# BowieHsu/tensorflow_ocr

Measured on AMD Instinct MI355X. Metric: images/sec training, 512x512 ICDAR, VGG-16 EAST, batch 32, 1/2/4/8 GPU, higher is better.
Workload: dtype f16; 1 GPU; VGG-16 model_vgg + dice loss train step, 512x512, batch 32 per GPU, f16 storage / f32 accumulate, Adam+EMA; global_batch=32, parallelism=dp1

## Files before the change

### include/ocr_hip.h

```cpp
#ifndef OCR_HIP_H_
#define OCR_HIP_H_

#include <stddef.h>
#include <stdint.h>

#ifdef __cplusplus
extern "C" {
#endif

#define OCR_ABI_VERSION 7

enum {
  OCR_OK = 0,
  OCR_ERR_INVALID_ARG = -1,
  OCR_ERR_UNSUPPORTED = -2,
  OCR_ERR_HIP = -3,
  OCR_ERR_WORKSPACE = -4,
  OCR_ERR_RCCL = -5
};

int ocr_abi_version(void);
const char* ocr_status_string(int status);
const char* ocr_storage_dtype(void);
uint32_t ocr_crc32c(const void* data, size_t n, uint32_t seed);
// ... 43 lines not shown

int ocr_conv2d_bnred_tail_f16(const ocr_conv_desc* d, const void* x, const void* w_kc, void* y, void* partial,
                              const void* bn_y, const void* bn_mean, const void* bn_invstd,
                              const void* tail_out, const void* tail_mask_bits, const void* sub_grad, void* stream);

int ocr_conv2d_pw_bnaddrelu_f16(const ocr_conv_desc* d, const void* prev_y, const void* prev_scale,
                                const void* prev_shift, const void* shortcut, const void* sc_scale,
                                const void* sc_shift, void* x_out, void* mask_bits, const void* w_kc, void* y,
                                void* stats, void* stream);
int ocr_conv2d_pw_bnrelu_f16(const ocr_conv_desc* d, const void* prev_y, const void* prev_scale, const void* prev_shift,
                             void* x_out, const void* w_kc, void* y, void* stats, void* stream);
int ocr_conv2d_pw_bnbwd_bnred_f16(const ocr_conv_desc* d, const void* dz, const void* y_above, const void* coef_a,
                                  const void* coef_b, const void* coef_c, void* dy_out, const void* w_kc, void* dx,
                                  void* partial, const void* bn_y, const void* bn_scale, const void* bn_shift,
                                  const void* bn_mean, const void* bn_invstd, int bn_relu, void* stream);
int ocr_conv2d_pw_bnbwd_tail_f16(const ocr_conv_desc* d, const void* dz, const void* y_above, const void* coef_a,
                                 const void* coef_b, const void* coef_c, const void* relu_shift, void* dy_out,
                                 const void* w_kc, void* dx, void* partial, const void* bn_y, const void* bn_mean,
                                 const void* bn_invstd, const void* tail_out, const void* tail_mask_bits,
                                 const void* sub_grad, void* stream);

int ocr_conv2d_first_f16(int n, int h, int w, int cout, const void* x4,
                         const void* w_first, const void* bias, int flags,
                         void* y, void* stats, void* stream);
int ocr_conv2d_first_num_mtiles(int n, int h, int w);

int ocr_conv2d_wgrad_f16(const ocr_conv_desc* d, const void* x, const void* dy,
                         void* dw_hwio_f32, void* workspace, size_t ws_bytes,
                         void* stream);
size_t ocr_conv2d_wgrad_workspace(const ocr_conv_desc* d);
int ocr_conv2d_wgrad_slabs_f16(const ocr_conv_desc* d, const void* x, const void* dy, void* workspace, size_t ws_bytes,
                               void* stream);
int ocr_conv2d_wgrad_reduce_f32(const ocr_conv_desc* d, const void* workspace, void* dw_hwio_f32, void* stream);
int ocr_conv2d_wgrad_guest_room(const ocr_conv_desc* d);

int ocr_conv2d_first_wgrad_f16(int n, int h, int w, int cout, const void* x4,
                               const void* dy, void* dw_hwio_f32,
                               void* workspace, size_t ws_bytes, void* stream);
int ocr_conv2d_first_wgrad_bn_f16(int n, int h, int w, int cout, const void* x4, const void* da, const void* bn_y,
                                  const void* w_first, const void* bn_shift, const void* coef_a, const void* coef_b,
                                  const void* coef_c, int relu, void* dw, void* workspace, size_t ws_bytes,
                                  void* stream);
int ocr_conv2d_first_bn_relu_f16(int n, int h, int w, int cout, const void* x4, const void* w_first,
                                 const void* scale, const void* shift, int relu, void* a, void* stream);
size_t ocr_conv2d_first_wgrad_workspace(int n, int h, int w, int cout);

int ocr_conv2d_stem_num_mtiles(int n, int h, int w);
int ocr_pack_weights_stem_f16(const void* w_hwio_f32, int cout, void* w_stem, void* stream);
int ocr_conv2d_stem_f16(int n, int h, int w, int cout, const void* x4, const void* w_stem,
                        const void* bias, int flags, void* y, void* stats, void* stream);
size_t ocr_conv2d_stem_wgrad_workspace(int n, int h, int w, int cout);
int ocr_conv2d_stem_wgrad_f16(int n, int h, int w, int cout, const void* x4, const void* dy,
                              void* dw_hwio_f32, void* workspace, size_t ws_bytes, void* stream);
int ocr_conv2d_stem_wgrad_bn_f16(int n, int h, int w, int cout, const void* x4, const void* da, const void* bn_y,
                                 const void* bn_shift, const void* coef_a, const void* coef_b, const void* coef_c,
                                 int relu, void* dw, void* workspace, size_t ws_bytes, void* stream);
int ocr_pack_weights_f16(const void* w_hwio_f32, int taps, int cin, int cout, void* w_kc,
                         void* w_ck, void* stream);
int ocr_pack_weights_first_f16(const void* w_hwio_f32, int cout, void* w_first, void* stream);
size_t ocr_conv2d_first_moments_workspace(void);
int ocr_conv2d_first_moments_f16(int n, int h, int w, int cout, const void* x4, const void* w_first, void* stats_row,
                                 void* workspace, size_t ws_bytes, void* stream);
int ocr_conv2d_first_moments_keep_f16(int n, int h, int w, int cout, const void* x4, const void* w_first,
                                      void* stats_row, void* moments_f64, void* workspace, size_t ws_bytes, void* stream);
size_t ocr_pack_weights_batch_table_bytes(int n);
int ocr_pack_weights_batch_table(int n, const void* const* w_hwio_f32, const int* taps, const int* cin,
// ... 344 lines not shown
```

### tensorflow_ocr_amd/csrc/conv_first.hip

```cpp
#include "common.h"
#include "conv_epilogue.h"

namespace {

constexpr int HW = 36;

struct FirstP {
  int n, h, w, cout, tiles_x, tiles_y, m_tiles, flags;
};

__device__ __forceinline__ void load_halo4(const half_t* __restrict__ x4, char* halo, int img, int h,
                                           int w, int iy0, int ix0) {
  for (int i = threadIdx.x; i < 10 * HW; i += 256) {
    const int hy = i / HW, hx = i - hy * HW;
    const int iy = iy0 + hy, ix = ix0 + hx;
    u32x2 v = {0u, 0u};
    if (iy >= 0 && iy < h && ix >= 0 && ix < w)
      v = *reinterpret_cast<const u32x2*>(x4 + (((size_t)img * h + iy) * w + ix) * 4);
    *reinterpret_cast<u32x2*>(halo + i * 8) = v;
  }
}

__device__ __forceinline__ void first_weights(const half_t* __restrict__ wf, int cout, int co0, int lane,
                                              half8_t (&a)[3][2]) {
  const int r = lane & 31, hh = lane >> 5;
#pragma unroll
  for (int ky = 0; ky < 3; ++ky)
#pragma unroll
    for (int i = 0; i < 2; ++i)
      a[ky][i] = *reinterpret_cast<const half8_t*>(wf + ((size_t)(ky * cout + co0 + i * 32 + r)) * 16 + 8 * hh);
}

__device__ __forceinline__ void first_mfma(const char* halo, const half8_t (&a)[3][2], int wave, int lane,
                                           f32x16 (&acc)[2][2]) {
  const int r = lane & 31, hh = lane >> 5;
#pragma unroll
  for (int i = 0; i < 2; ++i)
#pragma unroll
    for (int t = 0; t < 2; ++t)
#pragma unroll
      for (int e = 0; e < 16; ++e) acc[i][t][e] = 0.f;
#pragma unroll
  for (int ky = 0; ky < 3; ++ky) {
#pragma unroll
    for (int t = 0; t < 2; ++t) {
      const int ty = wave * 2 + t;
      const char* src = halo + ((ty + ky) * HW + r + 2 * hh) * 8;
      half4_t lo = *reinterpret_cast<const half4_t*>(src);
      half4_t hi = *reinterpret_cast<const half4_t*>(src + 8);
      half8_t b = {lo[0], lo[1], lo[2], lo[3], hi[0], hi[1], hi[2], hi[3]};
#pragma unroll
      for (int i = 0; i < 2; ++i)
        acc[i][t] = OCR_MFMA_32x32x16(a[ky][i], b, acc[i][t], 0, 0, 0);
    }
  }
}

struct FirstAct {
  const float *scale, *shift;
  int relu;
};

template <bool BNAPPLY>
// ... 556 lines not shown
```

### tensorflow_ocr_amd/csrc/conv_wgrad.hip

```cpp
#include "common.h"
#include <stdlib.h>

namespace ocr_detail {
int wgrad_pw_splits(const ocr_conv_desc* d);
int wgrad_pw_launch(const ocr_conv_desc* d, const void* x, const void* dy, void* slab, hipStream_t st);
bool wgrad_pw_is_256x256(const ocr_conv_desc* d);
}

namespace {

typedef short short4v __attribute__((__vector_size__(4 * sizeof(short))));
typedef __attribute__((address_space(3))) short4v* lds_s4_ptr;

struct WgP {
  int n, h, w, cin, oh, ow, cout, kh, kw, stride, dil, pt, pl;
  int tiles_x, tiles_y, m_tiles, HT, WT, splits, tiles_per_split, nci, nco;
};

OCR_DIAG_DECLARE(ocr_diag_wgrad)

constexpr int TILE_H = 8;
constexpr int TILE_W = 32;
constexpr int CIB = 64;
constexpr int COB = 64;
constexpr int XSTR = CIB * 2 + 16;
constexpr int DSTR = COB * 2 + 16;

__device__ __forceinline__ half8_t tr_pair(const char* base, int second_off) {
  short4v lo = __builtin_amdgcn_ds_read_tr16_b64_v4i16((lds_s4_ptr)(base));
  short4v hi = __builtin_amdgcn_ds_read_tr16_b64_v4i16((lds_s4_ptr)(base + second_off));
  typedef short short8v __attribute__((ext_vector_type(8)));
  short8v v = {lo[0], lo[1], lo[2], lo[3], hi[0], hi[1], hi[2], hi[3]};
  return __builtin_bit_cast(half8_t, v);
// ... 317 lines not shown
    }
    if (more) store_tile(buf ^ 1);
    __syncthreads();
  }

  OCR_DIAG_END(ocr_diag_wgrad)
#pragma unroll
  for (int t = 0; t < MAXTAPS; ++t) {
    if (t < ntaps) {
      float* dst = slab + (((size_t)(split * KG + kgrp) * ntaps + t) * p.cin + ci0 + ciw * 32 + 4 * g) * p.cout +
                   co0 + cow * 32 + li;
      if (ci0 + ciw * 32 < p.cin && co0 + cow * 32 < p.cout) {
#pragma unroll
        for (int i = 0; i < 2; ++i)
#pragma unroll
          for (int j = 0; j < 2; ++j)
#pragma unroll
            for (int e = 0; e < 4; ++e) dst[(size_t)(i * 16 + e) * p.cout + j * 16] = acc[t][i][j][e];
      }
    }
  }
}


template <int N> struct WgIC { static constexpr int value = N; };
template <typename F>
__device__ __forceinline__ void static_for4(F&& f) {
  f(WgIC<0>{});
  f(WgIC<1>{});
  f(WgIC<2>{});
  f(WgIC<3>{});
}

template <int MAXTAPS, int COB2>
__global__ __launch_bounds__(256) void wgrad3_kernel(Wg2P p, const half_t* __restrict__ x,
                                                      const half_t* __restrict__ dy,
                                                      float* __restrict__ slab) {
  constexpr int NT = 256;
  static_assert(COB2 == 128 || COB2 == 64, "cout block");
  constexpr int NJ = COB2 / 32;
  constexpr int DSTR2 = COB2 * 2 + 32;
  constexpr int DCH = COB2 / 8;
  constexpr int NDY = 128 * DCH / NT;
  constexpr int PPP = NT / DCH;
  constexpr int XPP = NT / 8;
  constexpr int NXMAX = (224 + XPP - 1) / XPP;
  extern __shared__ __attribute__((aligned(16))) char smem[];
  const int halo_px = p.HT * p.WT;
  const int halo_bytes = halo_px * X2STR;
  const int stage_bytes = halo_bytes + 128 * DSTR2;

  const int tid = threadIdx.x;
  const int lane = tid & 63, wave = tid >> 6;
  const int ciw = wave >> 1, cow = wave & 1;
  const int li = lane & 15, g = lane >> 4;
  const int q = li >> 2, pp = li & 3;

  int bid = blockIdx.x;
  if (p.xcd_swizzle) bid = (bid & 7) * (int)(gridDim.x >> 3) + (bid >> 3);
  const int cob = bid % p.nco;
  bid /= p.nco;
  const int cib = bid % p.nci;
  const int split = bid / p.nci;
  const int ci0 = cib * CIB, co0 = cob * COB2;
  const int ntaps = p.kh * p.kw;

  f32x4 acc[MAXTAPS][2][NJ];
#pragma unroll
  for (int t = 0; t < MAXTAPS; ++t)
#pragma unroll
    for (int i = 0; i < 2; ++i)
#pragma unroll
      for (int j = 0; j < NJ; ++j) acc[t][i][j] = f32x4{0.f, 0.f, 0.f, 0.f};

  const int a_lane = ((4 * g + q) * p.stride) * X2STR + (ciw * 32 + 4 * pp) * 2;
  const int a_half = 16 * p.stride * X2STR;
  const int b_lane = (4 * g + q) * DSTR2 + (cow * (COB2 / 2) + 4 * pp) * 2;
  const int b_half = 16 * DSTR2;

  const int mt_begin = split * p.tiles_per_split;
  int mt_end = mt_begin + p.tiles_per_split;
  if (mt_end > p.m_tiles) mt_end = p.m_tiles;

  constexpr unsigned OOB = 0xfffffff0u;
  constexpr int WT_ = 34, HALO_PX = 6 * WT_;
  const int xc = tid & 7;
  int hxv[NXMAX];
  unsigned relx[NXMAX];
#pragma unroll
  for (int u = 0; u < NXMAX; ++u) {
    const int hp = u * XPP + (tid >> 3);
    const int hy = hp / WT_, hx = hp - hy * WT_;
    hxv[u] = (hp < HALO_PX && ci0 + xc * 8 < p.cin) ? hx : 0x40000000;
    relx[u] = (unsigned)(((hy * p.w + hx) * p.cin + ci0 + xc * 8) * 2);
  }
  const int dc = tid % DCH, dprow = tid / DCH;
  int colv[2];
#pragma unroll
  for (int h2 = 0; h2 < 2; ++h2) colv[h2] = (co0 + dc * 8 < p.cout) ? (h2 * 16) % 32 + dprow : 0x40000000;
  const unsigned reld = (unsigned)((dprow * p.cout + co0 + dc * 8) * 2);

  int l_mt = mt_begin;
  int l_txi = l_mt % p.tiles_x, l_tyi = (l_mt / p.tiles_x) % p.tiles_y, l_img = l_mt / (p.tiles_x * p.tiles_y);
  int s_ix0 = 0, s_orgx = 0, s_ox0 = 0, s_orgd = 0;
  __amdgpu_buffer_rsrc_t xrs, drs;
  auto load_setup = [&]() {
    s_ix0 = l_txi * TILE_W - p.pl;
    s_orgx = ((l_tyi * T2_H - p.pt) * p.w + s_ix0) * p.cin * 2;
    s_ox0 = l_txi * TILE_W;
    s_orgd = ((l_tyi * T2_H) * p.ow + s_ox0) * p.cout * 2;
    xrs = __builtin_amdgcn_make_buffer_rsrc(const_cast<half_t*>(x) + (size_t)l_img * p.h * p.w * p.cin, 0,
                                            p.h * p.w * p.cin * 2, 0x00020000);
    drs = __builtin_amdgcn_make_buffer_rsrc(const_cast<half_t*>(dy) + (size_t)l_img * p.oh * p.ow * p.cout, 0,
                                            p.oh * p.ow * p.cout * 2, 0x00020000);
  };
  auto load_advance = [&]() {
    if (l_mt + 1 < mt_end) {
      ++l_mt;
      if (++l_txi == p.tiles_x) {
        l_txi = 0;
        if (++l_tyi == p.tiles_y) {
          l_tyi = 0;
          ++l_img;
        }
      }
    }
    load_setup();
  };
  u32x4 xr[NXMAX], dr[NDY];
  unsigned offp = 0;
  auto load_half = [&](int hh) {
    const int k = hh >> 1;
    if (k >= NXMAX + NDY) return;
    if (k < NXMAX) {
      if (!(hh & 1)) {
        const int ix = hxv[k] + s_ix0;
        offp = (unsigned)ix < (unsigned)p.w ? relx[k] + (unsigned)s_orgx : OOB;
      } else {
        xr[k] = __builtin_bit_cast(u32x4, __builtin_amdgcn_raw_buffer_load_b128(xrs, offp, 0, 0));
      }
    } else {
      const int u = k - NXMAX;
      if (!(hh & 1)) {
        const int ox = colv[((u * PPP) >> 4) & 1] + s_ox0;
        offp = (unsigned)ox < (unsigned)p.ow ? reld + (unsigned)(s_orgd + (((u * PPP) >> 5) * p.ow + ((u * PPP) & 31)) * p.cout * 2) : OOB;
      } else {
        dr[u] = __builtin_bit_cast(u32x4, __builtin_amdgcn_raw_buffer_load_b128(drs, offp, 0, 0));
      }
    }
  };
  auto store_piece = [&](int buf, int k) {
    char* xh = smem + buf * stage_bytes;
    if (k < NXMAX) {
      if (k * XPP + XPP <= HALO_PX || k * XPP + (tid >> 3) < HALO_PX)
        *reinterpret_cast<u32x4*>(xh + (k * XPP + (tid >> 3)) * X2STR + xc * 16) = xr[k];
    } else if (k < NXMAX + NDY) {
      const int u = k - NXMAX;
      *reinterpret_cast<u32x4*>(xh + halo_bytes + (u * PPP + dprow) * DSTR2 + dc * 16) = dr[u];
    }
  };
  auto load_tile = [&]() {
#pragma unroll
    for (int hh = 0; hh < 2 * (NXMAX + NDY); ++hh) load_half(hh);
  };
  auto store_tile = [&](int buf) {
#pragma unroll
    for (int k = 0; k < NXMAX + NDY; ++k) store_piece(buf, k);
  };

  OCR_DIAG_BEGIN()
  if (mt_begin < mt_end) {
    load_setup();
    load_tile();
    store_tile(0);
    load_advance();
    load_tile();
  }
  __syncthreads();
#ifndef WG3_ABL
#define WG3_ABL 0
#endif
  typedef short short8v __attribute__((ext_vector_type(8)));
  short4v al[4][2], ah[4][2], bl[2][NJ], bh[2][NJ];
  auto rd = [&](const char* a) { return __builtin_amdgcn_ds_read_tr16_b64_v4i16((lds_s4_ptr)(a)); };
  auto frag = [&](const short4v& lo, const short4v& hi) {
    short8v v = __builtin_shufflevector(lo, hi, 0, 1, 2, 3, 4, 5, 6, 7);
    return __builtin_bit_cast(half8_t, v);
  };
  auto read_b1 = [&](int set, const char* dyt, int ty, int k) {
    if constexpr ((WG3_ABL & 8) != 0) return;
    const char* a = dyt + b_lane + ty * 32 * DSTR2 + (k >> 1) * 32 + ((k & 1) ? b_half : 0);
    if (k & 1) bh[set][k >> 1] = rd(a);
    else bl[set][k >> 1] = rd(a);
  };
  auto read_a1 = [&](int slot, const char* xh, int ty, int t, int k) {
    if constexpr ((WG3_ABL & 4) != 0) return;
    const int ky = t / 3, kx = t - ky * 3;
    const char* a = xh + a_lane + ((ty + ky) * WT_ + kx) * X2STR + (k >> 1) * 32 + ((k & 1) ? a_half : 0);
    if (k & 1) ah[slot][k >> 1] = rd(a);
    else al[slot][k >> 1] = rd(a);
  };
  if (mt_begin < mt_end) {
#pragma unroll
    for (int k = 0; k < 2 * NJ; ++k) read_b1(0, smem + halo_bytes, 0, k);
#pragma unroll
    for (int k = 0; k < 4; ++k) {
      read_a1(0, smem, 0, 0, k);
      read_a1(1, smem, 0, 1, k);
    }
  }
  for (int mt = mt_begin; mt < mt_end; ++mt) {
    const int buf = (mt - mt_begin) & 1;
    const char* xh = smem + buf * stage_bytes;
    const char* dyt = xh + halo_bytes;
    const char* xh_n = smem + (buf ^ 1) * stage_bytes;
    static_for4([&](auto TY) {
      constexpr int ty = decltype(TY)::value;
      constexpr int S = ty & 1;
      if constexpr (ty == 1) {
        if constexpr (!(WG3_ABL & 2)) __builtin_amdgcn_s_barrier();
      }
      if constexpr (ty == 1) load_advance();
      if constexpr (ty == 2) {
        asm volatile("s_waitcnt lgkmcnt(0)" ::: "memory");
        if constexpr (!(WG3_ABL & 2)) __builtin_amdgcn_s_barrier();
      }
#pragma unroll
      for (int t = 0; t < 9; ++t) {
        const int t2 = t + 2;
        const int cur = (ty * 9 + t) & 3, nxt = (ty * 9 + t + 2) & 3;
#pragma unroll
        for (int i = 0; i < 2; ++i)
#pragma unroll
          for (int j = 0; j < NJ; ++j) {
            const half8_t fa = frag(al[cur][i], ah[cur][i]), fb = frag(bl[S][j], bh[S][j]);
            if (t < 8) mfma16_acc(acc[t][i][j], fa, fb);
            else if (ty == 3 && i == 1 && j == NJ - 1) mfma16_acc_v_drain(acc[t][i][j], fa, fb);
            else mfma16_acc_v(acc[t][i][j], fa, fb);
            const int m = i * NJ + j;
            if (m < 4) {
              if (t2 < 9) read_a1(nxt, xh, ty, t2, m);
              else if (ty < 3) read_a1(nxt, xh, ty + 1, t2 - 9, m);
              else read_a1(nxt, xh_n, 0, t2 - 9, m);
            }
            constexpr int FG = 4;
            const int fm = NJ == 4 ? m - 4 : m;
            if (fm >= 0) {
              constexpr int NBT = 2 * NJ / FG;
              if (t >= 4 && t < 4 + NBT) {
                const int k = (t - 4) * FG + fm;
                if (ty < 3) read_b1(S ^ 1, dyt, ty + 1, k);
                else read_b1(S ^ 1, xh_n + halo_bytes, 0, k);
              } else if constexpr (!(WG3_ABL & 1)) {
                constexpr int NPC = NXMAX + NDY, NSL = (9 - NBT) * FG;
                const int f = (t < 4 ? t : t - NBT) * FG + fm;
                if constexpr (ty == 1) {
                  if (f < NPC) store_piece(buf ^ 1, f);
                  else load_half(f - NPC);
                }
                if constexpr (ty == 2) load_half(f + NSL - NPC);
              }
            }
          }
      }
    });
  }
  OCR_DIAG_END(ocr_diag_wgrad)

#pragma unroll
  for (int t = 0; t < MAXTAPS; ++t) {
    if (t < ntaps) {
      float* dst = slab + (((size_t)split * ntaps + t) * p.cin + ci0 + ciw * 32 + 4 * g) * p.cout +
                   co0 + cow * (COB2 / 2) + li;
      if (ci0 + ciw * 32 < p.cin && co0 + cow * (COB2 / 2) < p.cout) {
#pragma unroll
        for (int i = 0; i < 2; ++i)
#pragma unroll
          for (int j = 0; j < NJ; ++j)
#pragma unroll
            for (int e = 0; e < 4; ++e) dst[(size_t)(i * 16 + e) * p.cout + j * 16] = acc[t][i][j][e];
      }
    }
  }
}

int fill2(const ocr_conv_desc* d, Wg2P* p, int* cob) {
  if (d->cin % 32 || d->cout % 32 || d->kh * d->kw > 9) return OCR_ERR_UNSUPPORTED;
  *cob = (d->cout % 128 == 0) ? 128 : 64;
  p->n = d->n; p->h = d->h; p->w = d->w; p->cin = d->cin;
  p->oh = d->oh; p->ow = d->ow; p->cout = d->cout;
  p->kh = d->kh; p->kw = d->kw; p->stride = d->stride; p->dil = d->dilation;
  p->pt = d->pad_top; p->pl = d->pad_left;
  p->tiles_x = ocr_cdiv(d->ow, TILE_W);
// ... 16 lines not shown
}

int fill(const ocr_conv_desc* d, WgP* p) {
  OCR_CHECK_ARG(d != nullptr);
  OCR_CHECK_ARG(d->n > 0 && d->h > 0 && d->w > 0 && d->oh > 0 && d->ow > 0);
  OCR_CHECK_SHAPE(d->cin % 64 == 0 && d->cout % 64 == 0);
  OCR_CHECK_SHAPE(d->kh * d->kw <= 9);
  p->n = d->n; p->h = d->h; p->w = d->w; p->cin = d->cin;
  p->oh = d->oh; p->ow = d->ow; p->cout = d->cout;
  p->kh = d->kh; p->kw = d->kw; p->stride = d->stride; p->dil = d->dilation;
  p->pt = d->pad_top; p->pl = d->pad_left;
  p->tiles_x = ocr_cdiv(d->ow, TILE_W);
  p->tiles_y = ocr_cdiv(d->oh, TILE_H);
  p->m_tiles = d->n * p->tiles_x * p->tiles_y;
  p->HT = (TILE_H - 1) * d->stride + (d->kh - 1) * d->dilation + 1;
  p->WT = (TILE_W - 1) * d->stride + (d->kw - 1) * d->dilation + 1;
  p->nci = d->cin / CIB;
  p->nco = d->cout / COB;
  const int blocks = p->nci * p->nco;
  int want = ocr_cdiv(1024, blocks);
  if (want > p->m_tiles) want = p->m_tiles;
  if (want < 1) want = 1;
  p->tiles_per_split = ocr_cdiv(p->m_tiles, want);
  p->splits = ocr_cdiv(p->m_tiles, p->tiles_per_split);
  size_t lds = (size_t)p->HT * p->WT * XSTR + 256 * DSTR;
  if (lds > 160 * 1024) return OCR_ERR_UNSUPPORTED;
  return OCR_OK;
}

}

OCR_DIAG_READER(ocr_diag_read_wgrad, ocr_diag_wgrad)

template <typename K, typename P>
static int launch_wg(K kern, const P& p, unsigned grid, size_t lds, const void* x, const void* dy,
                     void* ws, hipStream_t st, unsigned threads = 256) {
  if (hipFuncSetAttribute(reinterpret_cast<const void*>(kern),
                          hipFuncAttributeMaxDynamicSharedMemorySize, 160 * 1024) != hipSuccess)
    return OCR_ERR_HIP;
  hipLaunchKernelGGL(kern, dim3(grid), dim3(threads), lds, st, p, static_cast<const half_t*>(x),
                     static_cast<const half_t*>(dy), static_cast<float*>(ws));
  return ocr_launch_status();
}

struct WgradSel {
  enum Family { NONE, PW, TAP3, TAP2, GENERIC } family = NONE;
  int splits = 0;
  int cob = 0;
  Wg2P p2{};
  WgP p{};
};
static WgradSel wgrad_select(const ocr_conv_desc* d) {
  WgradSel s;
  if ((s.splits = ocr_detail::wgrad_pw_splits(d)) > 0) {
    s.family = WgradSel::PW;
    return s;
  }
  if (fill2(d, &s.p2, &s.cob) == OCR_OK) {
    static const int v3 = [] { const char* e = getenv("OCR_WGRAD3"); return e ? atoi(e) : 1; }();
    const bool small = (size_t)d->n * d->h * d->w * d->cin < (1u << 30) && (size_t)d->n * d->oh * d->ow * d->cout < (1u << 30);
    const bool use3 = d->kh * d->kw == 9 && v3 && small && d->cin % 64 == 0 && d->kw == 3 && d->stride == 1 && d->dilation == 1;
    s.family = use3 ? WgradSel::TAP3 : WgradSel::TAP2;
    s.splits = s.p2.splits * (s.cob == 64 && !use3 ? 2 : 1);
    return s;
  }
  if (fill(d, &s.p) == OCR_OK) {
    s.family = WgradSel::GENERIC;
    s.splits = s.p.splits * 2;
  }
  return s;
}

extern "C" size_t ocr_conv2d_wgrad_workspace(const ocr_conv_desc* d) {
  if (!d) return 0;
  return (size_t)wgrad_select(d).splits * d->kh * d->kw * d->cin * d->cout * sizeof(float);
}

static int wgrad_slabs(const ocr_conv_desc* d, const void* x, const void* dy, void* workspace, size_t ws_bytes,
                       void* stream, int* splits_out) {
  OCR_CHECK_ARG(d != nullptr);
  OCR_CHECK_ARG(d->n > 0 && d->h > 0 && d->w > 0 && d->oh > 0 && d->ow > 0);
  OCR_CHECK_ARG(x && dy && workspace);
  const size_t elems = (size_t)d->kh * d->kw * d->cin * d->cout;
  hipStream_t st = static_cast<hipStream_t>(stream);
  const int ntaps = d->kh * d->kw;
  WgradSel sel = wgrad_select(d);
  if (sel.family == WgradSel::NONE) return OCR_ERR_UNSUPPORTED;
  const int splits = sel.splits;
  if (ws_bytes < (size_t)splits * elems * sizeof(float)) return OCR_ERR_WORKSPACE;
  int rc;
  if (sel.family == WgradSel::PW) {
    rc = ocr_detail::wgrad_pw_launch(d, x, dy, workspace, st);
  } else if (sel.family == WgradSel::TAP3 || sel.family == WgradSel::TAP2) {
    Wg2P& p2 = sel.p2;
    const int cob = sel.cob;
    const size_t lds = 2 * ((size_t)p2.HT * p2.WT * X2STR + 128 * (cob * 2 + 32));
    const unsigned grid = (unsigned)(p2.splits * p2.nci * p2.nco);
    p2.xcd_swizzle = grid % 8 == 0;
    if (sel.family == WgradSel::TAP3)
      rc = cob == 128 ? launch_wg(wgrad3_kernel<9, 128>, p2, grid, lds, x, dy, workspace, st, 256)
                      : launch_wg(wgrad3_kernel<9, 64>, p2, grid, lds, x, dy, workspace, st, 256);
    else if (cob == 128)
      rc = ntaps == 1 ? launch_wg(wgrad2_kernel<128, 1>, p2, grid, lds, x, dy, workspace, st, 512)
                      : launch_wg(wgrad2_kernel<128, 9>, p2, grid, lds, x, dy, workspace, st, 512);
    else
      rc = ntaps == 1 ? launch_wg(wgrad2_kernel<64, 1>, p2, grid, lds, x, dy, workspace, st, 512)
                      : launch_wg(wgrad2_kernel<64, 9>, p2, grid, lds, x, dy, workspace, st, 512);
  } else {
    const WgP& p = sel.p;
    const size_t lds = (size_t)p.HT * p.WT * XSTR + 256 * DSTR;
    const unsigned grid = (unsigned)(p.splits * p.nci * p.nco);
    rc = ntaps == 1 ? launch_wg(wgrad_kernel<1>, p, grid, lds, x, dy, workspace, st, 512)
                    : launch_wg(wgrad_kernel<9>, p, grid, lds, x, dy, workspace, st, 512);
  }
  if (rc != OCR_OK) return rc;
  *splits_out = splits;
  return ocr_launch_status();
}

extern "C" int ocr_conv2d_wgrad_f16(const ocr_conv_desc* d, const void* x, const void* dy,
                                    void* dw, void* workspace, size_t ws_bytes, void* stream) {
  OCR_CHECK_ARG(dw != nullptr);
  int splits = 0;
  const int rc = wgrad_slabs(d, x, dy, workspace, ws_bytes, stream, &splits);
  if (rc != OCR_OK) return rc;
  const size_t elems4 = (size_t)d->kh * d->kw * d->cin * d->cout / 4;
  launch_slab_reduce(static_cast<const float*>(workspace), static_cast<float*>(dw), elems4, splits,
                     static_cast<hipStream_t>(stream));
  return ocr_launch_status();
}

extern "C" int ocr_conv2d_wgrad_slabs_f16(const ocr_conv_desc* d, const void* x, const void* dy, void* workspace,
                                          size_t ws_bytes, void* stream) {
  int splits = 0;
  return wgrad_slabs(d, x, dy, workspace, ws_bytes, stream, &splits);
}

static int wgrad_slab_count(const ocr_conv_desc* d) { return wgrad_select(d).splits; }

extern "C" int ocr_conv2d_wgrad_guest_room(const ocr_conv_desc* d) {
  if (!d || d->n <= 0 || d->h <= 0 || d->w <= 0 || d->oh <= 0 || d->ow <= 0) return 0;
  const WgradSel sel = wgrad_select(d);
  if (sel.family == WgradSel::PW) return ocr_detail::wgrad_pw_is_256x256(d) ? 80 : 0;
  if (sel.family != WgradSel::TAP3) return 0;
  return sel.cob == 128 ? 56 : 248;
}

extern "C" int ocr_conv2d_wgrad_reduce_f32(const ocr_conv_desc* d, const void* workspace, void* dw, void* stream) {
  OCR_CHECK_ARG(d && workspace && dw);
  OCR_CHECK_ARG(d->n > 0 && d->h > 0 && d->w > 0 && d->oh > 0 && d->ow > 0);
  const int splits = wgrad_slab_count(d);
  if (splits <= 0) return OCR_ERR_UNSUPPORTED;
  const size_t elems = (size_t)d->kh * d->kw * d->cin * d->cout;
  launch_slab_reduce(static_cast<const float*>(workspace), static_cast<float*>(dw), elems / 4, splits,
                     static_cast<hipStream_t>(stream));
  return ocr_launch_status();
}
```

### tensorflow_ocr_amd/layers.py

```python
import torch

from . import ops
from .graph import Act, F16, F32, constant, variance_scaling, xavier_uniform
from ._lib import CONV_ACCUM_F16, CONV_BIAS, CONV_RELU, CONV_STATS

BN_DECAY = 0.997
BN_EPS = 1e-5
FUSE_BN_REDUCE = __import__("os").environ.get("OCR_FUSE_BN", "1") == "1"


def _bn_vars(g, C):
    with g.variable_scope("BatchNorm"):
        gamma = g.get_variable("gamma", (C,), constant(1.0))
        beta = g.get_variable("beta", (C,), constant(0.0))
        mm = g.get_variable("moving_mean", (C,), constant(0.0), trainable=False)
        mv = g.get_variable("moving_variance", (C,), constant(1.0), trainable=False)
    return gamma, beta, mm, mv


def _packs(g, w, first):
    kh, kw, cin, cout = w.shape
    if first:
        def mk(old):
            t = old if old is not None else g.empty((3, cout, 16))
            ops.pack_weights_first(w.data, t)
            return t
        return g.packed(w, "first", mk), None

    def mk(old):
        if old is None:
            old = (g.empty((kh * kw, cout, cin)), g.empty((kh * kw, cin, cout)))
        ops.pack_weights(w.data, old[0], old[1])
        return old
    return g.packed(w, "kc_ck", mk)


FUSE_BIAS_POOL = __import__("os").environ.get("OCR_FUSE_BIAS_POOL", "1") == "1"
FUSE_BIAS_RELU = __import__("os").environ.get("OCR_FUSE_BIAS_RELU", "1") == "1"


def _const_vec(g, n, value):
    cache = g.__dict__.setdefault("_const_vecs", {})
    t = cache.get((n, value))
    if t is None:
        t = cache[(n, value)] = torch.full((n,), float(value), dtype=F32, device=g.device)
    return t


FUSE_BN_W4_MAXHW = int(__import__("os").environ.get("OCR_FUSE_BN_W4_MAXHW", "1000000"))
FUSE_BN_POOL_REDUCE = __import__("os").environ.get("OCR_FUSE_BN_POOL_REDUCE", "1") == "1"
FIRST_RECOMPUTE = __import__("os").environ.get("OCR_FIRST_RECOMPUTE", "1") == "1"
FIRST_DROP_Y = __import__("os").environ.get("OCR_FIRST_DROP_Y", "1") == "1"
FIRST_MOMENTS = __import__("os").environ.get("OCR_FIRST_MOMENTS", "1") == "1"
FIRST_WGRAD_RECOMPUTE = __import__("os").environ.get("OCR_FIRST_WGRAD_RECOMPUTE", "0") == "1"
GUEST_REDUCE = __import__("os").environ.get("OCR_GUEST_REDUCE", "1") == "1"
FUSE_FIRST_WGRAD = __import__("os").environ.get("OCR_FUSE_FIRST_WGRAD", "1") == "1"
FIRST_WGRAD_SUMS = __import__("os").environ.get("OCR_FIRST_WGRAD_SUMS", "1") == "1"


def conv2d(g, x, cout, k, scope, *, stride=1, rate=1, normalizer="bn", relu=True, pool=0,
           keep_full=True, is_training=True, bn_training=None, first=False, weight_decay=True,
           initializer=None):
    if g.precision == "f32":
        from . import layers_f32
        return layers_f32.conv2d(g, x, cout, k, scope, stride=stride, rate=rate, normalizer=normalizer,
                                 relu=relu, pool=pool, keep_full=keep_full, is_training=is_training,
                                 bn_training=bn_training, first=first, weight_decay=weight_decay,
                                 initializer=initializer)
    n, h, w, cin_x = x.shape
    cin = 3 if first else cin_x
    bn_training = is_training if bn_training is None else bn_training
    with g.variable_scope(scope):
        init = initializer or variance_scaling(g.rng)
        wv = g.get_variable("weights", (k, k, cin, cout), init, regularized=weight_decay)
        if normalizer == "bn":
            gamma, beta, mm, mv = _bn_vars(g, cout)
            bias = None
        else:
            bias = g.get_variable("biases", (cout,), constant(0.0))
    ws = g.workspace()
    w_fwd, w_dg = _packs(g, wv, first)
    if first:
        d = None
        oh, ow = h, w
        mt = ops.conv2d_first_num_mtiles(n, h, w)
    else:
        d = ops.conv_desc((n, h, w, cin), cout, k, k, stride, rate)
        oh, ow = d.oh, d.ow
        mt = ops.conv2d_num_mtiles(d)
    drop_y = (first and normalizer == "bn" and not pool and cout == 64 and FIRST_RECOMPUTE and FIRST_DROP_Y
# ... 174 lines not shown
    a_full = Act(y, name=scope)
    if relu and is_training:
        a_full.bias_ctx = (y, _const_vec(g, cout, 1.0), _const_vec(g, cout, 0.0), _const_vec(g, cout, 0.0),
                           _const_vec(g, cout, 1.0), True)

    def backward_bias():
        if a_full.grad is None:
            return
        if a_full.bias_done:
            dz = a_full.grad
            a_full.bias_done = False
        elif a_full.bias_partial is not None:
            part_f, T_f = a_full.bias_partial
            ops.bn_bwd_sums(part_f, T_f, cout, bias.grad, g.ws_small.get(cout * 4)[:cout * 4].view(F32), ws)
            dz = a_full.grad
            a_full.bias_partial = None
        else:
            dz = g.empty(y.shape)
            ops.bias_relu_bwd(y, a_full.grad, relu, dz, bias.grad, ws)
        _conv_backward(g, x, wv, w_dg, d, dz, first)
        a_full.grad = None
    g.record(backward_bias, (wv, bias))
    a_pool = max_pool2d(g, a_full, 2, 2, scope=scope + "/pool", bias_relu=bias if (relu and is_training) else None) if pool else None
    return a_full, a_pool


def _conv_backward(g, x, wv, w_dg, d, dy, first):
    ws = g.workspace()
    if first:
        ops.conv2d_first_wgrad(x.data, dy, wv.grad, ws)
        return
    dd = ops.ConvDesc(d.n, d.h, d.w, d.cin, d.oh, d.ow, d.cout, d.kh, d.kw, d.stride, d.dilation,
                      d.pad_top, d.pad_left, 0, 0)
    if ops.GUEST_BN and x.requires_grad:
        _conv_dgrad(g, x, wv, w_dg, d, dy)
        ops.conv2d_wgrad(dd, x.data, dy, wv.grad, g.ws_wgrad, alloc=lambda nb: g.empty((nb,), torch.uint8))
        return
    ops.conv2d_wgrad(dd, x.data, dy, wv.grad, g.ws_wgrad)
    if not x.requires_grad:
        return
    _conv_dgrad(g, x, wv, w_dg, d, dy)


def _conv_dgrad(g, x, wv, w_dg, d, dy):
    if d.stride != 1:
        raise NotImplementedError("strided dgrad")
    pt = d.dilation * (d.kh - 1) - d.pad_top
    pl = d.dilation * (d.kw - 1) - d.pad_left
    flags = 0
    by0 = x.bn_ctx[0] if x.bn_ctx is not None else None
    if (x.grad is None and x.sole_consumer and FIRST_WGRAD_SUMS and FUSE_BN_REDUCE and isinstance(by0, ops.LazyFirstY)
            and by0.t is None and by0.moments is not None and d.cin == 64):
        dg = ops.ConvDesc(d.n, d.oh, d.ow, d.cout, d.h, d.w, d.cin, d.kh, d.kw, 1, d.dilation, pt, pl, 1, 0)
        blocks = ops.conv2d_bnred_first_wgrad_blocks(dg)
        if blocks > 0:
            T = ops.conv2d_num_mtiles(dg)
            partial = g.empty((T, 2, d.cin), F32)
            s1 = g.empty((blocks, 32, 64), F32)
            ops.conv2d_bnred_first_wgrad(dg, dy, w_dg, partial, (by0.x4, by0.w_first) + tuple(x.bn_ctx[1:]), s1)
            x.bn_partial = (partial, T)
            x.first_s1 = s1
            return
    if x.grad is None:
        x.grad = g.empty(x.shape)
    else:
        flags |= CONV_ACCUM_F16
# ... 458 lines not shown
```

### tensorflow_ocr_amd/ops.py

```python
import ctypes
from ctypes import byref, c_double, c_float, c_int, c_int64, c_size_t

import torch

from . import _lib as L
from ._lib import ConvDesc, CONV_ACCUM_F16, CONV_BIAS, CONV_RELU, CONV_STATS, ptr

F16, F32 = (torch.bfloat16 if L.STORAGE == "bf16" else torch.float16), torch.float32


def _st():
    return L.stream_ptr()


def same_pad(size, k, stride, dilation=1):
    k_eff = (k - 1) * dilation + 1
    out = -(-size // stride)
    total = max((out - 1) * stride + k_eff - size, 0)
    return out, total // 2


class Workspace:

    def __init__(self, device, nbytes=64 << 20):
# ... 220 lines not shown
def bn_relu_bwd_apply_affine(y, da, scale, shift, coef_b, coef_c, relu, dy):
    n, h, w, c = y.shape
    L.call("ocr_bn_relu_bwd_apply_affine_f16", ptr(y), ptr(da), ptr(scale), ptr(shift), ptr(coef_b), ptr(coef_c),
           c_int(n), c_int(h), c_int(w), c_int(c), c_int(int(relu)), ptr(dy), c_int(0), _st())
    if L.RECORDER is not None:
        L.RECORDER.tag_last(("guest", 6.0 * n * h * w * c))


def bn_relu_pool_bwd_idx_apply_affine(y, argmax, da_pool, coef, relu, dy):
    n, h, w, c = y.shape
    L.call("ocr_bn_relu_pool_bwd_idx_apply_affine_f16", ptr(y), ptr(argmax), ptr(da_pool), ptr(coef[0]), ptr(coef[1]),
           ptr(coef[2]), c_int(n), c_int(h), c_int(w), c_int(c), c_int(int(relu)), ptr(dy), c_int(0), _st())
    if L.RECORDER is not None:
        L.RECORDER.tag_last(("guest", 4.75 * n * h * w * c))


def conv2d_wgrad(d, x, dy, dw, ws, alloc=None):
    nbytes = L.call_size("ocr_conv2d_wgrad_workspace", byref(d))
    flops = 2.0 * d.n * d.oh * d.ow * d.cout * d.cin * d.kh * d.kw
    if alloc is not None and GUEST_BN:
        buf = alloc(nbytes)
        L.call("ocr_conv2d_wgrad_slabs_f16", byref(d), ptr(x), ptr(dy), ptr(buf), c_size_t(nbytes), _st())
        if L.RECORDER is not None:
            room = L.call_int("ocr_conv2d_wgrad_guest_room", byref(d))
            L.RECORDER.tag_last(("side", flops) if room >= 56 else ("side",))
        L.call("ocr_conv2d_wgrad_reduce_f32", byref(d), ptr(buf), ptr(dw), _st())
        if L.RECORDER is not None:
            L.RECORDER.tag_last(("reduce",))
        return
    buf = ws.get(nbytes)
    L.call("ocr_conv2d_wgrad_f16", byref(d), ptr(x), ptr(dy), ptr(dw), ptr(buf), c_size_t(nbytes), _st())
    if L.RECORDER is not None:
        L.RECORDER.tag_last(("side",))


def space_to_depth(x, xs):
    n, h, w, c = x.shape
    L.call("ocr_space_to_depth_f16", ptr(x), c_int(n), c_int(h), c_int(w), c_int(c), ptr(xs), _st())


def depth_to_space(xs, x, accumulate):
    n, h, w, c = x.shape
    L.call("ocr_depth_to_space_f16", ptr(xs), c_int(n), c_int(h), c_int(w), c_int(c), ptr(x), c_int(int(accumulate)), _st())


def weights_s2d(w33, w22):
    _, _, cin, cout = w33.shape
    L.call("ocr_weights_s2d_f32", ptr(w33), c_int(cin), c_int(cout), ptr(w22), _st())


def weights_s2d_grad(dw22, dw33):
    _, _, cin, cout = dw33.shape
    L.call("ocr_weights_s2d_grad_f32", ptr(dw22), c_int(cin), c_int(cout), ptr(dw33), _st())
    if L.RECORDER is not None:
        L.RECORDER.tag_last(("side",))


def conv2d_first_num_mtiles(n, h, w):
    return L.call_int("ocr_conv2d_first_num_mtiles", c_int(n), c_int(h), c_int(w))


def conv2d_first(x4, w_first, y, flags=0, bias=None, stats=None, cout=None):
    n, h, w, _ = x4.shape
    cout = y.shape[-1] if y is not None else cout
    L.call("ocr_conv2d_first_f16", c_int(n), c_int(h), c_int(w), c_int(cout), ptr(x4), ptr(w_first),
           ptr(bias), c_int(flags), ptr(y), ptr(stats), _st())
# ... 764 lines not shown
```

Baseline: 1822 images/sec.

## Regenerate first-layer activations inside conv1_2 wgrad instead of reading them

Adds a variant of the 3x3 wgrad kernel for the second VGG conv (64->64) that recomputes its input activation on the fly. It loads the 4-channel image tile, runs the first conv via MFMA, and applies BN scale/shift and ReLU into the LDS halo, instead of reading a materialized 64-channel activation. This removes a large HBM read, and possibly the need to store that activation, in exchange for extra MFMA work and LDS traffic interleaved into the wgrad pipeline. The Python side routes to this path when the input is a lazy first-layer output and the shape is supported.

```diff
diff --git a/include/ocr_hip.h b/include/ocr_hip.h
--- a/include/ocr_hip.h
+++ b/include/ocr_hip.h
@@ -99,6 +99,10 @@
 int ocr_conv2d_wgrad_slabs_f16(const ocr_conv_desc* d, const void* x, const void* dy, void* workspace, size_t ws_bytes,
                                void* stream);
 int ocr_conv2d_wgrad_reduce_f32(const ocr_conv_desc* d, const void* workspace, void* dw_hwio_f32, void* stream);
+int ocr_conv2d_wgrad_first_supported(const ocr_conv_desc* d);
+int ocr_conv2d_wgrad_slabs_first_f16(const ocr_conv_desc* d, const void* x4, const void* w_first, const void* scale,
+                                     const void* shift, int relu, const void* dy, void* workspace, size_t ws_bytes,
+                                     void* stream);
 int ocr_conv2d_wgrad_guest_room(const ocr_conv_desc* d);
 
 int ocr_conv2d_first_wgrad_f16(int n, int h, int w, int cout, const void* x4,
diff --git a/tensorflow_ocr_amd/csrc/conv_first.hip b/tensorflow_ocr_amd/csrc/conv_first.hip
--- a/tensorflow_ocr_amd/csrc/conv_first.hip
+++ b/tensorflow_ocr_amd/csrc/conv_first.hip
@@ -1,5 +1,6 @@
 #include "common.h"
 #include "conv_epilogue.h"
+#include "conv_first_gen.h"
 
 namespace {
 
@@ -19,16 +20,6 @@
       v = *reinterpret_cast<const u32x2*>(x4 + (((size_t)img * h + iy) * w + ix) * 4);
     *reinterpret_cast<u32x2*>(halo + i * 8) = v;
   }
-}
-
-__device__ __forceinline__ void first_weights(const half_t* __restrict__ wf, int cout, int co0, int lane,
-                                              half8_t (&a)[3][2]) {
-  const int r = lane & 31, hh = lane >> 5;
-#pragma unroll
-  for (int ky = 0; ky < 3; ++ky)
-#pragma unroll
-    for (int i = 0; i < 2; ++i)
-      a[ky][i] = *reinterpret_cast<const half8_t*>(wf + ((size_t)(ky * cout + co0 + i * 32 + r)) * 16 + 8 * hh);
 }
 
 __device__ __forceinline__ void first_mfma(const char* halo, const half8_t (&a)[3][2], int wave, int lane,
diff --git a/tensorflow_ocr_amd/csrc/conv_first_gen.h b/tensorflow_ocr_amd/csrc/conv_first_gen.h
--- /dev/null
+++ b/tensorflow_ocr_amd/csrc/conv_first_gen.h
@@ -0,0 +1,45 @@
+#pragma once
+#include "common.h"
+
+namespace {
+
+__device__ __forceinline__ void first_weights(const half_t* __restrict__ wf, int cout, int co0, int lane,
+                                              half8_t (&a)[3][2]) {
+  const int r = lane & 31, hh = lane >> 5;
+#pragma unroll
+  for (int ky = 0; ky < 3; ++ky)
+#pragma unroll
+    for (int i = 0; i < 2; ++i)
+      a[ky][i] = *reinterpret_cast<const half8_t*>(wf + ((size_t)(ky * cout + co0 + i * 32 + r)) * 16 + 8 * hh);
+}
+
+__device__ __forceinline__ void first_mfma_block(const char* src, int pitch, const half8_t (&a)[3][2],
+                                                 f32x16 (&acc)[2]) {
+#pragma unroll
+  for (int i = 0; i < 2; ++i)
+#pragma unroll
+    for (int e = 0; e < 16; ++e) acc[i][e] = 0.f;
+#pragma unroll
+  for (int ky = 0; ky < 3; ++ky) {
+    half4_t lo = *reinterpret_cast<const half4_t*>(src + ky * pitch);
+    half4_t hi = *reinterpret_cast<const half4_t*>(src + ky * pitch + 8);
+    half8_t b = {lo[0], lo[1], lo[2], lo[3], hi[0], hi[1], hi[2], hi[3]};
+#pragma unroll
+    for (int i = 0; i < 2; ++i) acc[i] = OCR_MFMA_32x32x16(a[ky][i], b, acc[i], 0, 0, 0);
+  }
+}
+
+__device__ __forceinline__ half4_t first_act4(const f32x16& acc, int q, const f32x4& sc, const f32x4& sh, int relu,
+                                              bool inside) {
+  half4_t o;
+#pragma unroll
+  for (int e = 0; e < 4; ++e) {
+    const float y16 = (float)(half_t)acc[q * 4 + e];
+    float f = __builtin_fmaf(y16, sc[e], sh[e]);
+    if (relu) f = f > 0.f ? f : 0.f;
+    o[e] = inside ? (half_t)f : (half_t)0.f;
+  }
+  return o;
+}
+
+}
diff --git a/tensorflow_ocr_amd/csrc/conv_wgrad.hip b/tensorflow_ocr_amd/csrc/conv_wgrad.hip
--- a/tensorflow_ocr_amd/csrc/conv_wgrad.hip
+++ b/tensorflow_ocr_amd/csrc/conv_wgrad.hip
@@ -1,4 +1,5 @@
 #include "common.h"
+#include "conv_first_gen.h"
 #include <stdlib.h>
 
 namespace ocr_detail {
@@ -382,23 +383,35 @@
   f(WgIC<3>{});
 }
 
-template <int MAXTAPS, int COB2>
+struct WgNoGen {};
+struct WgGen {
+  const half_t* wf;
+  const float *scale, *shift;
+  int relu;
+};
+
+template <int MAXTAPS, int COB2, typename GP = WgNoGen>
 __global__ __launch_bounds__(256) void wgrad3_kernel(Wg2P p, const half_t* __restrict__ x,
                                                       const half_t* __restrict__ dy,
-                                                      float* __restrict__ slab) {
+                                                      float* __restrict__ slab, GP gp) {
   constexpr int NT = 256;
+  constexpr bool GEN = !__is_same(GP, WgNoGen);
   static_assert(COB2 == 128 || COB2 == 64, "cout block");
+  static_assert(!GEN || COB2 == 64, "the generated operand: cin = cout = 64");
   constexpr int NJ = COB2 / 32;
   constexpr int DSTR2 = COB2 * 2 + 32;
   constexpr int DCH = COB2 / 8;
   constexpr int NDY = 128 * DCH / NT;
   constexpr int PPP = NT / DCH;
   constexpr int XPP = NT / 8;
-  constexpr int NXMAX = (224 + XPP - 1) / XPP;
+  constexpr int NXMAX = GEN ? 2 : (224 + XPP - 1) / XPP;
+  constexpr int IW = 38, IMG_PX = 8 * IW, IPITCH = IW * 8;
   extern __shared__ __attribute__((aligned(16))) char smem[];
   const int halo_px = p.HT * p.WT;
   const int halo_bytes = halo_px * X2STR;
   const int stage_bytes = halo_bytes + 128 * DSTR2;
+  char* const imgt = smem + 2 * stage_bytes;
+  char* const bnv = imgt + IMG_PX * 8;
 
   const int tid = threadIdx.x;
   const int lane = tid & 63, wave = tid >> 6;
@@ -439,10 +452,32 @@
   unsigned relx[NXMAX];
 #pragma unroll
   for (int u = 0; u < NXMAX; ++u) {
-    const int hp = u * XPP + (tid >> 3);
-    const int hy = hp / WT_, hx = hp - hy * WT_;
-    hxv[u] = (hp < HALO_PX && ci0 + xc * 8 < p.cin) ? hx : 0x40000000;
-    relx[u] = (unsigned)(((hy * p.w + hx) * p.cin + ci0 + xc * 8) * 2);
+    if constexpr (GEN) {
+      const int ip = u * NT + tid;
+      const int iy = ip / IW, ix = ip - iy * IW;
+      hxv[u] = ip < IMG_PX ? ix : 0x40000000;
+      relx[u] = (unsigned)((iy * p.w + ix) * 8);
+    } else {
+      const int hp = u * XPP + (tid >> 3);
+      const int hy = hp / WT_, hx = hp - hy * WT_;
+      hxv[u] = (hp < HALO_PX && ci0 + xc * 8 < p.cin) ? hx : 0x40000000;
+      relx[u] = (unsigned)(((hy * p.w + hx) * p.cin + ci0 + xc * 8) * 2);
+    }
+  }
+  half8_t gw[GEN ? 3 : 1][2];
+  int g_src[2], g_dst[2], g_pos[2];
+  if constexpr (GEN) {
+    first_weights(gp.wf, 64, 0, lane, gw);
+    if (tid < 128) reinterpret_cast<float*>(bnv)[tid] = tid < 64 ? gp.scale[tid] : gp.shift[tid - 64];
+#pragma unroll
+    for (int j = 0; j < 2; ++j) {
+      const int hp = (wave + 4 * j) * 32 + (lane & 31);
+      const int hpc = hp < HALO_PX ? hp : HALO_PX - 1;
+      const int hy = hpc / WT_, hx = hpc - hy * WT_;
+      g_src[j] = (hy * IW + hx + 2 * (lane >> 5)) * 8;
+      g_dst[j] = hp < HALO_PX ? hp * X2STR : -1;
+      g_pos[j] = (hy << 16) | hx;
+    }
   }
   const int dc = tid % DCH, dprow = tid / DCH;
   int colv[2];
@@ -452,15 +487,23 @@
 
   int l_mt = mt_begin;
   int l_txi = l_mt % p.tiles_x, l_tyi = (l_mt / p.tiles_x) % p.tiles_y, l_img = l_mt / (p.tiles_x * p.tiles_y);
-  int s_ix0 = 0, s_orgx = 0, s_ox0 = 0, s_orgd = 0;
+  int s_ix0 = 0, s_orgx = 0, s_ox0 = 0, s_orgd = 0, s_iy0 = 0;
   __amdgpu_buffer_rsrc_t xrs, drs;
   auto load_setup = [&]() {
     s_ix0 = l_txi * TILE_W - p.pl;
-    s_orgx = ((l_tyi * T2_H - p.pt) * p.w + s_ix0) * p.cin * 2;
     s_ox0 = l_txi * TILE_W;
     s_orgd = ((l_tyi * T2_H) * p.ow + s_ox0) * p.cout * 2;
+    if constexpr (GEN) {
+      s_iy0 = l_tyi * T2_H - p.pt;
+      s_ix0 -= 1;
+      s_orgx = ((s_iy0 - 1) * p.w + s_ix0) * 8;
+      xrs = __builtin_amdgcn_make_buffer_rsrc(const_cast<half_t*>(x) + (size_t)l_img * p.h * p.w * 4, 0, p.h * p.w * 8,
+                                              0x00020000);
+    } else {
+    s_orgx = ((l_tyi * T2_H - p.pt) * p.w + s_ix0) * p.cin * 2;
     xrs = __builtin_amdgcn_make_buffer_rsrc(const_cast<half_t*>(x) + (size_t)l_img * p.h * p.w * p.cin, 0,
                                             p.h * p.w * p.cin * 2, 0x00020000);
+    }
     drs = __builtin_amdgcn_make_buffer_rsrc(const_cast<half_t*>(dy) + (size_t)l_img * p.oh * p.ow * p.cout, 0,
                                             p.oh * p.ow * p.cout * 2, 0x00020000);
   };
@@ -477,7 +520,8 @@
     }
     load_setup();
   };
-  u32x4 xr[NXMAX], dr[NDY];
+  u32x4 xr[GEN ? 1 : NXMAX], dr[NDY];
+  u32x2 xi[GEN ? NXMAX : 1];
   unsigned offp = 0;
   auto load_half = [&](int hh) {
     const int k = hh >> 1;
@@ -487,7 +531,8 @@
         const int ix = hxv[k] + s_ix0;
         offp = (unsigned)ix < (unsigned)p.w ? relx[k] + (unsigned)s_orgx : OOB;
       } else {
-        xr[k] = __builtin_bit_cast(u32x4, __builtin_amdgcn_raw_buffer_load_b128(xrs, offp, 0, 0));
+        if constexpr (GEN) xi[k] = __builtin_bit_cast(u32x2, __builtin_amdgcn_raw_buffer_load_b64(xrs, offp, 0, 0));
+        else xr[k] = __builtin_bit_cast(u32x4, __builtin_amdgcn_raw_buffer_load_b128(xrs, offp, 0, 0));
       }
     } else {
       const int u = k - NXMAX;
@@ -502,7 +547,9 @@
   auto store_piece = [&](int buf, int k) {
     char* xh = smem + buf * stage_bytes;
     if (k < NXMAX) {
-      if (k * XPP + XPP <= HALO_PX || k * XPP + (tid >> 3) < HALO_PX)
+      if constexpr (GEN) {
+        if (k * NT + NT <= IMG_PX || k * NT + tid < IMG_PX) *reinterpret_cast<u32x2*>(imgt + (k * NT + tid) * 8) = xi[k];
+      } else if (k * XPP + XPP <= HALO_PX || k * XPP + (tid >> 3) < HALO_PX)
         *reinterpret_cast<u32x4*>(xh + (k * XPP + (tid >> 3)) * X2STR + xc * 16) = xr[k];
     } else if (k < NXMAX + NDY) {
       const int u = k - NXMAX;
@@ -518,11 +565,40 @@
     for (int k = 0; k < NXMAX + NDY; ++k) store_piece(buf, k);
   };
 
+  f32x16 gacc[GEN ? 2 : 1][2];
+  int g_iy0 = 0, g_ix0 = 0;
+  auto gen_part = [&](char* xh, int j) {
+    if constexpr (GEN) {
+      if (j >= 18) return;
+      const int b = j < 2 ? j : (j - 2) >> 3;
+      if (b == 1 && __builtin_amdgcn_readfirstlane(wave) == 3) return;
+      if (j < 2) {
+        first_mfma_block(imgt + g_src[b], IPITCH, gw, gacc[b]);
+      } else {
+        const int i = ((j - 2) >> 2) & 1, q = (j - 2) & 3;
+        const int c0 = i * 32 + q * 8 + (lane >> 5) * 4;
+        const f32x4 sc = *reinterpret_cast<const f32x4*>(bnv + c0 * 4);
+        const f32x4 sh = *reinterpret_cast<const f32x4*>(bnv + (64 + c0) * 4);
+        const bool inside = (unsigned)(g_iy0 + (g_pos[b] >> 16)) < (unsigned)p.h &&
+                            (unsigned)(g_ix0 + (g_pos[b] & 0xffff)) < (unsigned)p.w;
+        const half4_t o = first_act4(gacc[b][i], q, sc, sh, gp.relu, inside);
+        if (g_dst[b] >= 0) *reinterpret_cast<half4_t*>(xh + g_dst[b] + c0 * 2) = o;
+      }
+    }
+  };
   OCR_DIAG_BEGIN()
   if (mt_begin < mt_end) {
     load_setup();
     load_tile();
     store_tile(0);
+    if constexpr (GEN) {
+      g_iy0 = s_iy0;
+      g_ix0 = s_ix0 + 1;
+      __syncthreads();
+#pragma unroll
+      for (int j = 0; j < 18; ++j) gen_part(smem, j);
+      __syncthreads();
+    }
     load_advance();
     load_tile();
   }
@@ -568,7 +644,12 @@
       constexpr int ty = decltype(TY)::value;
       constexpr int S = ty & 1;
       if constexpr (ty == 1) {
+        if constexpr (GEN) asm volatile("s_waitcnt lgkmcnt(0)" ::: "memory");
         if constexpr (!(WG3_ABL & 2)) __builtin_amdgcn_s_barrier();
+      }
+      if constexpr (ty == 1 && GEN) {
+        g_iy0 = s_iy0;
+        g_ix0 = s_ix0 + 1;
       }
       if constexpr (ty == 1) load_advance();
       if constexpr (ty == 2) {
@@ -604,11 +685,24 @@
               } else if constexpr (!(WG3_ABL & 1)) {
                 constexpr int NPC = NXMAX + NDY, NSL = (9 - NBT) * FG;
                 const int f = (t < 4 ? t : t - NBT) * FG + fm;
+                if constexpr (GEN) {
+                  constexpr int NGP = 18;
+                  if constexpr (ty == 0) {
+                    if (f < NXMAX) store_piece(buf ^ 1, f);
+                  }
+                  if constexpr (ty == 1) {
+                    gen_part(smem + (buf ^ 1) * stage_bytes, f);
+                    if (f < NDY) store_piece(buf ^ 1, NXMAX + f);
+                    if (f >= NGP) load_half(f - NGP);
+                  }
+                  if constexpr (ty == 2) load_half(f + NSL - NGP);
+                } else {
                 if constexpr (ty == 1) {
                   if (f < NPC) store_piece(buf ^ 1, f);
                   else load_half(f - NPC);
                 }
                 if constexpr (ty == 2) load_half(f + NSL - NPC);
+                }
               }
             }
           }
@@ -691,14 +785,14 @@
 
 OCR_DIAG_READER(ocr_diag_read_wgrad, ocr_diag_wgrad)
 
-template <typename K, typename P>
+template <typename K, typename P, typename... Extra>
 static int launch_wg(K kern, const P& p, unsigned grid, size_t lds, const void* x, const void* dy,
-                     void* ws, hipStream_t st, unsigned threads = 256) {
+                     void* ws, hipStream_t st, unsigned threads = 256, Extra... extra) {
   if (hipFuncSetAttribute(reinterpret_cast<const void*>(kern),
                           hipFuncAttributeMaxDynamicSharedMemorySize, 160 * 1024) != hipSuccess)
     return OCR_ERR_HIP;
   hipLaunchKernelGGL(kern, dim3(grid), dim3(threads), lds, st, p, static_cast<const half_t*>(x),
-                     static_cast<const half_t*>(dy), static_cast<float*>(ws));
+                     static_cast<const half_t*>(dy), static_cast<float*>(ws), extra...);
   return ocr_launch_status();
 }
 
@@ -757,8 +851,8 @@
     const unsigned grid = (unsigned)(p2.splits * p2.nci * p2.nco);
     p2.xcd_swizzle = grid % 8 == 0;
     if (sel.family == WgradSel::TAP3)
-      rc = cob == 128 ? launch_wg(wgrad3_kernel<9, 128>, p2, grid, lds, x, dy, workspace, st, 256)
-                      : launch_wg(wgrad3_kernel<9, 64>, p2, grid, lds, x, dy, workspace, st, 256);
+      rc = cob == 128 ? launch_wg(wgrad3_kernel<9, 128>, p2, grid, lds, x, dy, workspace, st, 256, WgNoGen{})
+                      : launch_wg(wgrad3_kernel<9, 64>, p2, grid, lds, x, dy, workspace, st, 256, WgNoGen{});
     else if (cob == 128)
       rc = ntaps == 1 ? launch_wg(wgrad2_kernel<128, 1>, p2, grid, lds, x, dy, workspace, st, 512)
                       : launch_wg(wgrad2_kernel<128, 9>, p2, grid, lds, x, dy, workspace, st, 512);
@@ -795,6 +889,33 @@
   return wgrad_slabs(d, x, dy, workspace, ws_bytes, stream, &splits);
 }
 
+static bool wgrad_first_ok(const ocr_conv_desc* d, const WgradSel& sel) {
+  return sel.family == WgradSel::TAP3 && sel.cob == 64 && d->cin == 64 && d->cout == 64 && d->kh == 3 && d->pad_top == 1 &&
+         d->pad_left == 1 && d->oh == d->h && d->ow == d->w && (size_t)d->h * d->w * 8 < (1u << 31);
+}
+extern "C" int ocr_conv2d_wgrad_first_supported(const ocr_conv_desc* d) {
+  if (!d || d->n <= 0 || d->h <= 0 || d->w <= 0 || d->oh <= 0 || d->ow <= 0) return 0;
+  return wgrad_first_ok(d, wgrad_select(d)) ? 1 : 0;
+}
+extern "C" int ocr_conv2d_wgrad_slabs_first_f16(const ocr_conv_desc* d, const void* x4, const void* w_first,
+                                                const void* scale, const void* shift, int relu, const void* dy,
+                                                void* workspace, size_t ws_bytes, void* stream) {
+  OCR_CHECK_ARG(d != nullptr);
+  OCR_CHECK_ARG(d->n > 0 && d->h > 0 && d->w > 0 && d->oh > 0 && d->ow > 0);
+  OCR_CHECK_ARG(x4 && w_first && scale && shift && dy && workspace);
+  WgradSel sel = wgrad_select(d);
+  if (!wgrad_first_ok(d, sel)) return OCR_ERR_UNSUPPORTED;
+  const size_t elems = (size_t)d->kh * d->kw * d->cin * d->cout;
+  if (ws_bytes < (size_t)sel.splits * elems * sizeof(float)) return OCR_ERR_WORKSPACE;
+  Wg2P& p2 = sel.p2;
+  const size_t lds = 2 * ((size_t)p2.HT * p2.WT * X2STR + 128 * (64 * 2 + 32)) + 8 * 38 * 8 + 2 * 64 * sizeof(float);
+  const unsigned grid = (unsigned)(p2.splits * p2.nci * p2.nco);
+  p2.xcd_swizzle = grid % 8 == 0;
+  return launch_wg(wgrad3_kernel<9, 64, WgGen>, p2, grid, lds, x4, dy, workspace, static_cast<hipStream_t>(stream), 256,
+                   WgGen{static_cast<const half_t*>(w_first), static_cast<const float*>(scale),
+                         static_cast<const float*>(shift), relu});
+}
+
 static int wgrad_slab_count(const ocr_conv_desc* d) { return wgrad_select(d).splits; }
 
 extern "C" int ocr_conv2d_wgrad_guest_room(const ocr_conv_desc* d) {
diff --git a/tensorflow_ocr_amd/layers.py b/tensorflow_ocr_amd/layers.py
--- a/tensorflow_ocr_amd/layers.py
+++ b/tensorflow_ocr_amd/layers.py
@@ -56,6 +56,7 @@
 GUEST_REDUCE = __import__("os").environ.get("OCR_GUEST_REDUCE", "1") == "1"
 FUSE_FIRST_WGRAD = __import__("os").environ.get("OCR_FUSE_FIRST_WGRAD", "1") == "1"
 FIRST_WGRAD_SUMS = __import__("os").environ.get("OCR_FIRST_WGRAD_SUMS", "1") == "1"
+FIRST_GEN_WGRAD = __import__("os").environ.get("OCR_FIRST_GEN_WGRAD", "1") == "1"
 
 
 def conv2d(g, x, cout, k, scope, *, stride=1, rate=1, normalizer="bn", relu=True, pool=0,
@@ -296,6 +297,17 @@
         return
     dd = ops.ConvDesc(d.n, d.h, d.w, d.cin, d.oh, d.ow, d.cout, d.kh, d.kw, d.stride, d.dilation,
                       d.pad_top, d.pad_left, 0, 0)
+    by0 = x.bn_ctx[0] if x.bn_ctx is not None else None
+    if FIRST_GEN_WGRAD and isinstance(by0, ops.LazyFirstY) and ops.conv2d_wgrad_first_supported(dd):
+        first_ctx = (by0.x4, by0.w_first, x.bn_ctx[1], x.bn_ctx[2], x.bn_ctx[5])
+        if ops.GUEST_BN and x.requires_grad:
+            _conv_dgrad(g, x, wv, w_dg, d, dy)
+            ops.conv2d_wgrad_first(dd, first_ctx, dy, wv.grad, g.ws_wgrad, alloc=lambda nb: g.empty((nb,), torch.uint8))
+            return
+        ops.conv2d_wgrad_first(dd, first_ctx, dy, wv.grad, g.ws_wgrad)
+        if x.requires_grad:
+            _conv_dgrad(g, x, wv, w_dg, d, dy)
+        return
     if ops.GUEST_BN and x.requires_grad:
         _conv_dgrad(g, x, wv, w_dg, d, dy)
         ops.conv2d_wgrad(dd, x.data, dy, wv.grad, g.ws_wgrad, alloc=lambda nb: g.empty((nb,), torch.uint8))
diff --git a/tensorflow_ocr_amd/ops.py b/tensorflow_ocr_amd/ops.py
--- a/tensorflow_ocr_amd/ops.py
+++ b/tensorflow_ocr_amd/ops.py
@@ -276,6 +276,25 @@
     L.call("ocr_conv2d_wgrad_f16", byref(d), ptr(x), ptr(dy), ptr(dw), ptr(buf), c_size_t(nbytes), _st())
     if L.RECORDER is not None:
         L.RECORDER.tag_last(("side",))
+
+
+def conv2d_wgrad_first_supported(d):
+    return bool(L.call_int("ocr_conv2d_wgrad_first_supported", byref(d)))
+
+
+def conv2d_wgrad_first(d, first_ctx, dy, dw, ws, alloc=None):
+    x4, wf, sc, sh, relu = first_ctx
+    nbytes = L.call_size("ocr_conv2d_wgrad_workspace", byref(d))
+    flops = 2.0 * d.n * d.oh * d.ow * d.cout * d.cin * d.kh * d.kw
+    split = alloc is not None and GUEST_BN
+    buf = alloc(nbytes) if split else ws.get(nbytes)
+    L.call("ocr_conv2d_wgrad_slabs_first_f16", byref(d), ptr(x4), ptr(wf), ptr(sc), ptr(sh), c_int(int(relu)), ptr(dy),
+           ptr(buf), c_size_t(nbytes), _st())
+    if L.RECORDER is not None:
+        L.RECORDER.tag_last(("side", flops) if split else ("side",))
+    L.call("ocr_conv2d_wgrad_reduce_f32", byref(d), ptr(buf), ptr(dw), _st())
+    if L.RECORDER is not None:
+        L.RECORDER.tag_last(("reduce",) if split else ("side",))
 
 
 def space_to_depth(x, xs):
```

Result: slower. 1750 images/sec (-3.9%).
